# kartikmadhira1/YA_VO

Hardware: AMD Instinct MI355X
Metric: frames/sec (detect+describe+match+PnP) on 1241×376 KITTI stereo; RMSE vs CPU ref (higher is better)
Workload: dtype u8

## Files before the change

### ya_vo_amd/csrc/yavo_kernels.hip

```cpp
#include <hip/hip_runtime.h>
#include <stdint.h>
#include <stdlib.h>
#include <string.h>

#include <algorithm>

#include "yavo_xlane.h"
#include "yavo_internal.h"


namespace yavo {

__device__ __forceinline__ int lane_id() { return (int)(threadIdx.x & 63); }

__device__ __forceinline__ int wave_incl_scan(int v) {
    v += __builtin_amdgcn_update_dpp(0, v, 0x111, 0xf, 0xf, false);
    v += __builtin_amdgcn_update_dpp(0, v, 0x112, 0xf, 0xf, false);
    v += __builtin_amdgcn_update_dpp(0, v, 0x114, 0xf, 0xf, false);
    v += __builtin_amdgcn_update_dpp(0, v, 0x118, 0xf, 0xf, false);
    v += __builtin_amdgcn_update_dpp(0, v, 0x142, 0xa, 0xf, false);
    v += __builtin_amdgcn_update_dpp(0, v, 0x143, 0xc, 0xf, false);
    return v;
}

// ... 54 lines not shown
    float d0 = m00 / scale, d1 = m11 / scale, e = m01 / scale;
    int iter = 0, ok = 1;
    while (true) {
        if (fabsf(e) < 1.17549435082228750797e-38f) {
            e = 0.0f;
        } else {
            const float se = 8388608.0f * e;
            if (se * se <= (fabsf(d0) + fabsf(d1))) e = 0.0f;
        }
        if (e == 0.0f) break;
        if (++iter > 60) { ok = 0; break; }
        const float td = (d0 - d1) * 0.5f;
        float mu = d1;
        if (td == 0.0f) {
            mu -= fabsf(e);
        } else {
            const float e2 = e * e;
            const float h = eig_hypotf(td, e);
            if (e2 == 0.0f) mu -= e / ((td + (td > 0.0f ? h : -h)) / e);
            else mu -= e2 / (td + (td > 0.0f ? h : -h));
        }
        const float x = d0 - mu, z = e;
        float c, sn;
        if (x == 0.0f) {
            c = 0.0f;
            sn = z < 0.0f ? 1.0f : -1.0f;
        } else if (fabsf(x) > fabsf(z)) {
            const float t = z / x;
            float u = sqrtf(1.0f + t * t);
            if (x < 0.0f) u = -u;
            c = 1.0f / u;
            sn = -t * c;
        } else {
            const float t = x / z;
            float u = sqrtf(1.0f + t * t);
            if (z < 0.0f) u = -u;
            sn = -1.0f / u;
            c = -t * sn;
        }
        const float sdk = sn * d0 + c * e;
        const float dkp1 = sn * e + c * d1;
        const float nd0 = c * (c * d0 - sn * e) - sn * (c * e - sn * d1);
        const float nd1 = sn * sdk + c * dkp1;
        const float ne = c * sdk - sn * dkp1;
        d0 = nd0;
        d1 = nd1;
        e = ne;
    }
    if (ok && d1 < d0) { const float t = d0; d0 = d1; d1 = t; }
    d0 *= scale;
    d1 *= scale;
    w0 = d1;
    w1 = d0;
}

__device__ __forceinline__ float harris_response(float a, float b, float d, int eig) {
    float w0 = a, w1 = d;
    if (eig == 1) {
        eig_selfadjoint2(a, b, d, w0, w1);
    } else if (!(fabsf(b) <= 1.1920928955078125e-07f)) {
        const float p = b;
        const float y = (float)((double)(w1 - w0) * 0.5);
        float t = fabsf(y) + cv_hypotf(p, y);
        float s = cv_hypotf(p, t);
        s = p / s;
        t = (p / t) * p;
        if (y < 0.0f) { s = -s; t = -t; }
        w0 -= t;
        w1 += t;
    }
    if (eig != 1 && w0 < w1) { float tmp = w0; w0 = w1; w1 = tmp; }
    const float prod = w0 * w1;
    const float sum = w1 + w0;
    const double sq = (double)sum * (double)sum;
    const double r = (double)prod - 0.04 * sq;
    return (float)r;
}

__device__ __forceinline__ uint64_t make_key(float resp, uint32_t idx) {
    if (resp == 0.0f) resp = 0.0f;
    uint32_t u = __float_as_uint(resp);
    uint32_t ord = (u & 0x80000000u) ? ~u : (u | 0x80000000u);
    return ((uint64_t)(~ord) << 32) | (uint64_t)idx;
}
__device__ __forceinline__ float key_resp(uint64_t key) {
    uint32_t ord = ~(uint32_t)(key >> 32);
    uint32_t u = (ord & 0x80000000u) ? (ord & 0x7fffffffu) : ~ord;
    return __uint_as_float(u);
}

struct K9 {
    uint32_t k[9];
    uint32_t kh[4][3];
    int hbias;
};

static K9 make_k9(const uint16_t* k9) {
    K9 kw = {};
    uint32_t sum = 0;
    for (int i = 0; i < 9; ++i) {
        kw.k[i] = k9[i];
        sum += k9[i];
    }
    auto tap = [&](int t) -> uint32_t { return (t >= 0 && t <= 8) ? (uint32_t)k9[t] : 0u; };
    for (int j = 0; j < 4; ++j)
        for (int m = 0; m < 3; ++m)
            for (int i = 0; i < 4; ++i) kw.kh[j][m] |= tap(4 * m + i - j) << (8 * i);
    kw.hbias = (int)(128 * sum);
    return kw;
}

__device__ __forceinline__ int reflect101(int p, int len) {
    if (p < 0) p = -p;
    if (p >= len) p = 2 * len - p - 2;
    return p;
}

#ifdef YAVO_LM_PROFILE
constexpr int kDetProfSlots = 131072;
__device__ unsigned long long g_det_prof[kDetProfSlots][6];
#define DP_DECL unsigned long long dp_acc[6] = {0, 0, 0, 0, 0, 0}; unsigned long long dp_t = __builtin_readcyclecounter();
#define DP_MARK(k) do { const unsigned long long t_ = __builtin_readcyclecounter(); dp_acc[k] += t_ - dp_t; dp_t = t_; } while (0)
#define DP_STORE() do { \
        const unsigned slot_ = blockIdx.x; \
        if (threadIdx.x == 0 && slot_ < kDetProfSlots) for (int q_ = 0; q_ < 6; ++q_) g_det_prof[slot_][q_] = dp_acc[q_]; \
    } while (0)
constexpr int kBriefProfSlots = 16384;
__device__ unsigned long long g_brief_prof[kBriefProfSlots][6];
#define BP_DECL unsigned long long bp_acc[3] = {0, 0, 0}; unsigned long long bp_t = __builtin_readcyclecounter(); \
    unsigned long long bp_bands = 0; const unsigned long long bp_rt0 = __builtin_amdgcn_s_memrealtime();
#define BP_MARK(k) do { const unsigned long long t_ = __builtin_readcyclecounter(); bp_acc[k] += t_ - bp_t; bp_t = t_; } while (0)
#define BP_BAND() do { ++bp_bands; } while (0)
#define BP_STORE() do { \
        if (threadIdx.x == 0 && blockIdx.x < kBriefProfSlots) { \
            g_brief_prof[blockIdx.x][0] = bp_acc[0]; g_brief_prof[blockIdx.x][1] = bp_acc[1]; \
            g_brief_prof[blockIdx.x][2] = bp_rt0; \
            g_brief_prof[blockIdx.x][3] = __builtin_amdgcn_s_memrealtime(); \
            g_brief_prof[blockIdx.x][4] = (unsigned long long)__builtin_amdgcn_s_getreg(0xF804) | (bp_bands << 32); \
            g_brief_prof[blockIdx.x][5] = (unsigned long long)__builtin_amdgcn_s_getreg(0xF814) | (bp_acc[2] << 32); \
        } \
    } while (0)
#else
#define DP_DECL
#define DP_MARK(k) do {} while (0)
#define DP_STORE() do {} while (0)
#define BP_DECL
#define BP_MARK(k) do {} while (0)
#define BP_BAND() do {} while (0)
#define BP_STORE() do {} while (0)
#endif
constexpr int FT_W = kFastTileW;
constexpr int FT_H = kFastTileH;
constexpr int FT_R = 4;
constexpr int FT_LW = FT_W + 2 * FT_R;
constexpr int FT_LH = FT_H + 2 * FT_R;
constexpr int kBandM = 19;
constexpr int kBlurStageDw = FT_LH * (FT_W / 4);

__device__ __forceinline__ void blur_tile_mfma(const uint8_t* tile, const uint32_t* s_band, uint32_t* stage, int hbias,
                                               int lane, int cb) {
    typedef int dt_v4i __attribute__((ext_vector_type(4)));
    const int nn = lane & 15, g = lane >> 4;
    const uint32_t* band = &s_band[(nn & 3) * kBandM + 3 - (nn >> 2)];
    const dt_v4i B = {(int)band[4 * g], (int)band[4 * g + 1], (int)band[4 * g + 2], (int)band[4 * g + 3]};
    const dt_v4i Z = {0, 0, 0, 0};
    const uint8_t* arow = &tile[nn * FT_LW + 16 * cb + 16 * g];
    dt_v4i Hlo, Hhi;
#pragma unroll
    for (int rb = 0; rb < 4; ++rb) {
        const uint2 lo = *reinterpret_cast<const uint2*>(arow + 16 * rb * FT_LW);
        const uint2 hi = *reinterpret_cast<const uint2*>(arow + 16 * rb * FT_LW + 8);
        const dt_v4i A = {(int)(lo.x ^ 0x80808080u), (int)(lo.y ^ 0x80808080u), (int)(hi.x ^ 0x80808080u),
                          (int)(hi.y ^ 0x80808080u)};
        const dt_v4i acc = __builtin_amdgcn_mfma_i32_16x16x64_i8(A, B, Z, 0, 0, 0);
        const uint32_t p01 = __builtin_amdgcn_perm((uint32_t)acc[1], (uint32_t)acc[0], 0x05010400u);
        const uint32_t p23 = __builtin_amdgcn_perm((uint32_t)acc[3], (uint32_t)acc[2], 0x05010400u);
        Hlo[rb] = (int)(__builtin_amdgcn_perm(p23, p01, 0x05040100u) ^ 0x80808080u);
        Hhi[rb] = (int)__builtin_amdgcn_perm(p23, p01, 0x07060302u);
    }
    const int T0 = (int)band[g], T1 = (int)band[g + 4];
    const int cv = 257 * hbias + (1 << 15);
    const dt_v4i Cv = {cv, cv, cv, cv};
    uint32_t* ostage = &stage[nn * 16 + ((4 * cb) ^ (nn & 12)) + g];
#pragma unroll
    for (int ob = 0; ob < 4; ++ob) {
        dt_v4i T = {0, 0, 0, 0};
        T[ob] = T0;
        if (ob < 3) T[ob + 1] = T1;
        const dt_v4i vl = __builtin_amdgcn_mfma_i32_16x16x64_i8(Hlo, T, Cv, 0, 0, 0);
        const dt_v4i vh = __builtin_amdgcn_mfma_i32_16x16x64_i8(Hhi, T, Z, 0, 0, 0);
        uint32_t v[4];
#pragma unroll
        for (int i = 0; i < 4; ++i) v[i] = ((uint32_t)vh[i] << 8) + (uint32_t)vl[i];
        ostage[ob * 16 * 16] = __builtin_amdgcn_perm(__builtin_amdgcn_perm(v[3], v[2], 0x0c0c0602u),
                                                     __builtin_amdgcn_perm(v[1], v[0], 0x0c0c0602u), 0x05040100u);
    }
}

__device__ __forceinline__ void blur_store_rows(const uint32_t* stage, uint8_t* __restrict__ blur, int img, int H, int W,
                                                int r0, int c0, int tid) {
    if (tid < FT_H * 4) {
        const int R = tid >> 2, q = tid & 3;
        const int bp = blur_pitch(W);
        if (r0 + R < H)
            *reinterpret_cast<uint4*>(blur + ((int64_t)img * H + r0 + R) * bp + c0 + 16 * (q ^ ((R >> 2) & 3))) =
                *reinterpret_cast<const uint4*>(&stage[R * 16 + 4 * q]);
    }
}

template <bool kBlur>
__global__ __launch_bounds__(256) void detect_kernel(const uint8_t* __restrict__ imgs, int H, int W, int stride,
                                                     int64_t pitch, int thr, int eig, uint64_t* __restrict__ cand_keys,
                                                     int64_t cap, uint32_t* __restrict__ cand_count, K9 kw,
                                                     uint8_t* __restrict__ blur) {
    __shared__ __align__(16) uint8_t tile[FT_LH * FT_LW];
    constexpr int kPreDw = FT_W * FT_H / 2;
    static_assert(kBlurStageDw <= kPreDw, "the blur's output staging must fit in the pretest list");
    __shared__ __align__(16) uint32_t s_share[kPreDw];
    uint16_t* s_pre = reinterpret_cast<uint16_t*>(s_share);
    __shared__ uint16_t s_pos[FT_W * FT_H];
    __shared__ uint32_t s_n, s_npre, s_base;
    __shared__ uint32_t s_band[4 * kBandM];
    DP_DECL
    const int ntx = (W + FT_W - 1) / FT_W, nty = (H + FT_H - 1) / FT_H;
    const int lb = xcd_swizzle((int)blockIdx.x, (int)gridDim.x);
    const int img = lb / (ntx * nty), tyx = lb - img * (ntx * nty);
    const int r0 = (tyx / ntx) * FT_H, c0 = (tyx % ntx) * FT_W;
    const uint8_t* src = imgs + (int64_t)img * pitch;
    const int tid = threadIdx.x;
    const int lane = lane_id();
    const int wave = tid >> 6;
    if (tid == 0) {
        s_n = 0;
        s_npre = 0;
    }
    if (kBlur && tid < 4 * kBandM) {
        const int r = tid / kBandM, M = tid - kBandM * r - 3;
        uint32_t v = 0;
#pragma unroll
        for (int j = 0; j < 4; ++j)
#pragma unroll
            for (int m = 0; m < 3; ++m)
                if (r == j && M == m) v = kw.kh[j][m];
        s_band[tid] = v;
    }

    {
        constexpr int kDw = FT_LW / 4;
        constexpr int kSlots = FT_LH * kDw;
        constexpr int kPer = (kSlots + 255) / 256;
        const bool interior = (c0 >= FT_R) && (c0 + FT_W + FT_R <= W) && (r0 >= FT_R) && (r0 + FT_H + FT_R < H);
        uint32_t v[kPer];
        if (interior) {
            const uint8_t* base = src + (int64_t)(r0 - FT_R) * stride + (c0 - FT_R);
            const int lr0 = tid / kDw, j0 = tid - lr0 * kDw;
            uint32_t off = (uint32_t)(lr0 * stride + 4 * j0);
            int j = j0;
            const uint32_t step = (uint32_t)(14 * stride + 16), wrap = (uint32_t)(15 * stride - 56);
            const uint32_t last = (uint32_t)((kSlots - 1) / kDw * stride + 4 * ((kSlots - 1) % kDw));
#pragma unroll
            for (int u = 0; u < kPer; ++u) {
                const uint32_t o = (256 * u + 255 >= kSlots && tid + 256 * u >= kSlots) ? last : off;
                __builtin_memcpy(&v[u], base + o, 4);
                const bool c = j + 4 >= kDw;
                off += c ? wrap : step;
                j += c ? 4 - kDw : 4;
            }
        } else {
#pragma unroll
            for (int u = 0; u < kPer; ++u) {
                const int t = min(tid + 256 * u, kSlots - 1);
                const int lr = t / kDw, j = t - lr * kDw;
                const int r = reflect101(min(max(r0 - FT_R + lr, -(H - 1)), 2 * H - 2), H);
                const uint8_t* row = src + (int64_t)r * stride;
                const int cc = c0 - FT_R + 4 * j;
                if (cc >= 0 && cc + 4 <= W) {
                    __builtin_memcpy(&v[u], row + cc, 4);
                } else {
                    uint32_t w = 0;
#pragma unroll
                    for (int b = 0; b < 4; ++b)
                        w |= (uint32_t)row[reflect101(min(max(cc + b, -(W - 1)), 2 * W - 2), W)] << (8 * b);
                    v[u] = w;
                }
            }
        }
        uint32_t* tile32 = reinterpret_cast<uint32_t*>(tile);
#pragma unroll
        for (int u = 0; u < kPer; ++u) {
            const int t = tid + 256 * u;
            if (t < kSlots) tile32[t] = v[u];
        }
    }
    __syncthreads();
    DP_MARK(0);

    constexpr int ring_dr[16] = YV_RING_DR;
    constexpr int ring_dc[16] = YV_RING_DC;
    const uint32_t neg_thr = (uint32_t)(-thr);
    const int tx = lane;
    const int ty = __builtin_amdgcn_readfirstlane(wave);
    const int c = c0 + tx;
    constexpr int kRowIters = FT_H / 4;
    uint32_t row_ok = 0;
#pragma unroll
    for (int u = 0; u < kRowIters; ++u) row_ok |= (uint32_t)((unsigned)(r0 + ty + 4 * u - 4) < (unsigned)(H - 8)) << u;
    uint32_t nmask = 0;
    const uint8_t* wbase = &tile[(ty + FT_R - 3) * FT_LW + tx + FT_R - 3];
#pragma unroll
    for (int u = kRowIters - 1; u >= 0; --u) {
        const uint8_t* t0 = wbase + 4 * u * FT_LW;
        const uint32_t cent = t0[3 * FT_LW + 3];
        auto d = [&](int k) {
            return __builtin_amdgcn_sad_u8(cent, (uint32_t)t0[(ring_dr[k] + 3) * FT_LW + ring_dc[k] + 3], neg_thr);
        };
        const uint32_t v = (d(0) | d(4)) | (d(8) | d(11));
        nmask = __builtin_amdgcn_alignbit(nmask, v, 31);
    }
    uint32_t pmask = (unsigned)(c - 4) < (unsigned)(W - 8) ? (~nmask & row_ok) : 0u;
    {
        const int cnt = __popc(pmask);
        const int incl = wave_incl_scan(cnt);
        const int total = __shfl(incl, 63, 64);
        uint32_t base = 0;
        if (lane == 0 && total > 0) base = atomicAdd(&s_npre, (uint32_t)total);
        base = __shfl(base, 0, 64);
        uint32_t off = base + (uint32_t)(incl - cnt);
        while (pmask) {
            const int u = __builtin_ctz(pmask);
            s_pre[off++] = (uint16_t)((ty + 4 * u) * FT_W + tx);
            pmask &= pmask - 1;
        }
    }
    __syncthreads();
    DP_MARK(1);
    const uint32_t npre = s_npre;
    for (uint32_t i0 = 0; i0 < npre; i0 += 256) {
        const uint32_t i = i0 + tid;
        bool cand = false;
        int pos = 0;
        if (i < npre) {
            pos = s_pre[i];
            const uint8_t* t0 = &tile[((pos >> 6) + FT_R - 3) * FT_LW + (pos & 63) + FT_R - 3];
            const uint32_t cent = t0[3 * FT_LW + 3];
            uint32_t sim = 0;
#pragma unroll
            for (int k = 0; k < 16; ++k)
                sim = __builtin_amdgcn_alignbit(
                    sim, __builtin_amdgcn_sad_u8(cent, (uint32_t)t0[(ring_dr[k] + 3) * FT_LW + ring_dc[k] + 3], neg_thr),
                    31);
            const uint32_t mask = ~sim & 0xFFFFu;
            const uint32_t a2 = mask & (mask >> 1);
            const uint32_t a4 = a2 & (a2 >> 2);
            const uint32_t a8 = a4 & (a4 >> 4);
            const uint32_t a12 = a8 & (a4 >> 8);
            cand = a12 != 0u;
        }
        const uint64_t bal = __ballot(cand);
        if (bal == 0) continue;
        const int leader = __ffsll((long long)bal) - 1;
        uint32_t base = 0;
        if (lane == leader) base = atomicAdd(&s_n, (uint32_t)__popcll(bal));
        base = __shfl(base, leader, 64);
        if (cand) s_pos[base + (uint32_t)__popcll(bal & ((1ull << lane) - 1ull))] = (uint16_t)pos;
    }
    __syncthreads();
    DP_MARK(2);
    const uint32_t n = s_n;
    auto harris = [&](uint32_t base) {
        uint64_t* out = cand_keys + (int64_t)img * cap + base;
        for (uint32_t i = tid; i < n; i += 256) {
            const int pos = s_pos[i];
            const int prr = pos >> 6, ptx = pos & 63;
            const uint8_t* t0 = &tile[(prr + FT_R - 2) * FT_LW + ptx + FT_R - 2];
            int sxx = 0, sxy = 0, syy = 0;
#pragma unroll
            for (int ii = -1; ii <= 1; ++ii) {
#pragma unroll
                for (int j = -1; j <= 1; ++j) {
                    const uint8_t* q = t0 + (ii + 2) * FT_LW + j + 2;
                    const int pmm = q[-FT_LW - 1], pm0 = q[-FT_LW], pmp = q[-FT_LW + 1];
                    const int p0m = q[-1], p0p = q[1];
                    const int ppm = q[FT_LW - 1], pp0 = q[FT_LW], ppp = q[FT_LW + 1];
                    const int gx = (pmp - pmm) + 2 * (p0p - p0m) + (ppp - ppm);
                    const int gy = (ppm - pmm) + 2 * (pp0 - pm0) + (ppp - pmp);
                    sxx += gx * gx;
                    sxy += gx * gy;
                    syy += gy * gy;
                }
            }
            const float resp = harris_response((float)sxx, (float)sxy, (float)syy, eig);
            out[i] = make_key(resp, (uint32_t)((r0 + prr) * W + (c0 + ptx)));
        }
    };
    if (tid == 0 && n > 0) s_base = atomicAdd(&cand_count[img], n);
    if constexpr (kBlur) blur_tile_mfma(tile, s_band, s_share, kw.hbias, lane, ty);
    __syncthreads();
    if constexpr (kBlur) blur_store_rows(s_share, blur, img, H, W, r0, c0, tid);
    DP_MARK(3);
    if (n > 0) harris(s_base);
    DP_MARK(4);
    DP_STORE();
}

void launch_fast_harris(const uint8_t* imgs, int n_images, int H, int W, int stride, int64_t pitch,
                        int thr, int eig, uint64_t* cand_keys, int64_t cap, uint32_t* cand_count, hipStream_t s) {
    dim3 grid(((W + FT_W - 1) / FT_W) * ((H + FT_H - 1) / FT_H) * n_images);
    K9 kw = {};
    hipLaunchKernelGGL(detect_kernel<false>, grid, dim3(256), 0, s, imgs, H, W, stride, pitch, thr, eig, cand_keys,
                       cap, cand_count, kw, (uint8_t*)nullptr);
}

void launch_detect_blur(const uint8_t* imgs, int n_images, int H, int W, int stride, int64_t pitch, int thr,
                        int eig, uint64_t* cand_keys, int64_t cap, uint32_t* cand_count, const uint16_t* k9_host,
                        uint8_t* blur, hipStream_t s) {
    uint32_t max_tap = 0;
    for (int i = 0; i < 9; ++i) max_tap = k9_host[i] > max_tap ? k9_host[i] : max_tap;
    if (max_tap > 127) {
        launch_fast_harris(imgs, n_images, H, W, stride, pitch, thr, eig, cand_keys, cap, cand_count, s);
        launch_blur9(imgs, n_images, H, W, stride, pitch, k9_host, blur, s);
        return;
    }
    dim3 grid(((W + FT_W - 1) / FT_W) * ((H + FT_H - 1) / FT_H) * n_images);
    const K9 kw = make_k9(k9_host);
    hipLaunchKernelGGL(detect_kernel<true>, grid, dim3(256), 0, s, imgs, H, W, stride, pitch, thr, eig, cand_keys, cap,
                       cand_count, kw, blur);
}

constexpr int BL_W = 64, BL_H = 32, BL_R = 4;
constexpr int BL_LW = BL_W + 2 * BL_R;
constexpr int BL_LH = BL_H + 2 * BL_R;

__global__ __launch_bounds__(256) void blur9_kernel(const uint8_t* __restrict__ imgs, int H, int W, int stride,
                                                    int64_t pitch, K9 kw, uint8_t* __restrict__ blur) {
    __shared__ uint8_t tin[BL_LH * BL_LW];
    __shared__ uint32_t th[BL_LH * BL_W];
    const int img = blockIdx.z;
    const int r0 = blockIdx.y * BL_H, c0 = blockIdx.x * BL_W;
    const uint8_t* src = imgs + (int64_t)img * pitch;
    const int tid = threadIdx.x;
    for (int i = tid; i < BL_LH * BL_LW; i += 256) {
        const int lr = i / BL_LW, lc = i - lr * BL_LW;
        const int r = reflect101(min(max(r0 - BL_R + lr, -(H - 1)), 2 * H - 2), H);
        const int c = reflect101(min(max(c0 - BL_R + lc, -(W - 1)), 2 * W - 2), W);
        tin[i] = src[(int64_t)r * stride + c];
    }
    __syncthreads();
    for (int i = tid; i < BL_LH * BL_W; i += 256) {
        const int lr = i >> 6, lc = i & 63;
        const uint8_t* q = &tin[lr * BL_LW + lc];
        uint32_t acc = 0;
#pragma unroll
        for (int j = 0; j < 9; ++j) acc += kw.k[j] * (uint32_t)q[j];
        th[i] = acc;
    }
    __syncthreads();
    const int tx = tid & 63, ty = tid >> 6;
    const int c = c0 + tx;
    for (int rr = ty; rr < BL_H; rr += 4) {
        const int r = r0 + rr;
        uint32_t acc = 0;
#pragma unroll
        for (int i = 0; i < 9; ++i) acc += kw.k[i] * th[(rr + i) * BL_W + tx];
        uint32_t v = (acc + (1u << 15)) >> 16;
        if (r < H && c < W) blur[(int64_t)img * blur_image_bytes(H, W) + (int64_t)r * blur_pitch(W) + c] = (uint8_t)(v > 255u ? 255u : v);
    }
}

void launch_blur9(const uint8_t* imgs, int n_images, int H, int W, int stride, int64_t pitch,
                  const uint16_t* k9_host, uint8_t* blur, hipStream_t s) {
    const K9 kw = make_k9(k9_host);
    constexpr int kMaxGridZ = 65535;
    for (int i0 = 0; i0 < n_images; i0 += kMaxGridZ) {
        const int n = n_images - i0 < kMaxGridZ ? n_images - i0 : kMaxGridZ;
        dim3 grid((W + BL_W - 1) / BL_W, (H + BL_H - 1) / BL_H, n);
        hipLaunchKernelGGL(blur9_kernel, grid, dim3(256), 0, s, imgs + (int64_t)i0 * pitch, H, W, stride, pitch, kw,
                           blur + (int64_t)i0 * blur_image_bytes(H, W));
    }
}

constexpr int TK_NT = 1024;

__device__ __forceinline__ bool brief_boundary(int row, int col, int H, int W) {
    return !(col - 8 < 0 || col + 8 > W) && !(row - 8 < 0 || row + 8 > H);
}

__host__ __device__ constexpr int bank_classes(int nb) { return nb <= kBandCounters / 32 ? 32 : 1; }

template <int NT, class RcAt>
__device__ void boundary_compact(RcAt rc_at, int K, int H, int W, int32_t* kp_src, int32_t* kp_count,
                                 int32_t* kp_band, int32_t* band_off, int* s_tmp, int* s_band) {
    const int tid = threadIdx.x;
    const int nb = (H + kBandRows - 1) / kBandRows;
    const int C = bank_classes(nb), nbc = nb * C;
    const int LS = brief_lds_stride(W);
    auto bucket = [&](int row, int col) -> int {
        const int band = row / kBandRows;
        const int cls = C == 1 ? 0 : ((((row - band * kBandRows + 8) * LS + col) >> 2) & 31);
        return band * C + cls;
    };
    for (int b = tid; b < nbc; b += NT) s_band[b] = 0;
    __syncthreads();
    int base = 0;
    for (int pass = 0; pass < 2; ++pass) {
        base = 0;
        for (int c0 = 0; c0 < K; c0 += 4 * NT) {
            int flags[4];
            int2 rcs[4];
            int cnt = 0;
#pragma unroll
            for (int u = 0; u < 4; ++u) {
                const int i = c0 + tid * 4 + u;
                flags[u] = 0;
                rcs[u] = make_int2(0, 0);
                if (i < K) {
                    rcs[u] = rc_at(i);
                    flags[u] = brief_boundary(rcs[u].x, rcs[u].y, H, W) ? 1 : 0;
                }
                cnt += flags[u];
            }
            int total = 0;
            int off = base + block_excl_scan<NT>(cnt, s_tmp, &total);
#pragma unroll
            for (int u = 0; u < 4; ++u) {
                const int i = c0 + tid * 4 + u;
                if (flags[u]) {
                    const int bk = bucket(rcs[u].x, rcs[u].y);
                    if (pass == 0) {
                        reinterpret_cast<int4*>(kp_src)[off] = make_int4(rcs[u].x, rcs[u].y, i, 0);
                        atomicAdd(&s_band[bk], 1);
                    } else {
                        const int pos = atomicAdd(&s_band[bk], 1);
                        reinterpret_cast<int4*>(kp_band)[pos] = make_int4(rcs[u].x, rcs[u].y, i, off);
                    }
                    off++;
                }
            }
            base += total;
        }
        __syncthreads();
        if (pass == 0) {
            int acc = 0;
            for (int b0 = 0; b0 < nbc; b0 += NT) {
                const int j = b0 + tid;
                const int c = j < nbc ? s_band[j] : 0;
                int tot = 0;
                const int first = acc + block_excl_scan<NT>(c, s_tmp, &tot);
                if (j < nbc) {
                    s_band[j] = first;
                    if (j % C == 0) band_off[j / C] = first;
                }
                acc += tot;
            }
            if (tid == 0) band_off[nb] = acc;
        }
        __syncthreads();
    }
    if (tid == 0) *kp_count = base;
}

constexpr int TK_SEL_NT = 512;
static_assert(TK_SEL_NT >= 256 && TK_SEL_NT % 64 == 0, "the radix-select histogram scan uses the first 256 threads");
template <int NT>
__global__ __launch_bounds__(NT) void topk_kernel(const uint64_t* __restrict__ cand_keys, int64_t cap,
                                                     uint32_t* __restrict__ cand_count, uint32_t* __restrict__ cand_seen,
                                                     int H, int W, int max_kp, int keep, int32_t* __restrict__ det_rc,
                                                     float* __restrict__ det_resp, int32_t* __restrict__ det_count,
                                                     int32_t* __restrict__ kp_src, int32_t* __restrict__ kp_count,
                                                     int32_t* __restrict__ kp_band, int32_t* __restrict__ band_off,
                                                     int32_t* __restrict__ brief_heads) {
    __shared__ uint64_t s_keys[kMaxKp];
    __shared__ uint32_t s_hist[256];
    __shared__ int s_tmp[40];
    __shared__ int s_band[kBandCounters];
    __shared__ uint64_t s_prefix, s_mask;
    __shared__ int s_krem, s_done, s_n;

    const int img = blockIdx.x;
    const int tid = threadIdx.x;
    if (img == 0 && tid < kBriefHeads) brief_heads[tid] = 0;
    const uint64_t* keys = cand_keys + (int64_t)img * cap;
    int64_t C64 = (int64_t)cand_count[img];
    if (C64 > cap) C64 = cap;
    const int C = (int)C64;
    const int K = C < keep ? C : keep;
    __syncthreads();
    if (tid == 0) {
        cand_seen[img] = (uint32_t)C;
        cand_count[img] = 0;
    }
    int32_t* rc_out = det_rc + (int64_t)img * max_kp * 2;
    float* resp_out = det_resp + (int64_t)img * max_kp;

    if (K == 0) {
        const int nb = (H + kBandRows - 1) / kBandRows;
        for (int b = tid; b <= nb; b += NT) band_off[(int64_t)img * (kMaxBands + 1) + b] = 0;
        if (tid == 0) { det_count[img] = 0; kp_count[img] = 0; }
        return;
    }
    uint64_t sel_mask = 0, sel_prefix = ~0ull;
    if (C > K) {
        if (tid == 0) { s_prefix = 0; s_mask = 0; s_krem = K; s_done = 0; }
        __syncthreads();
        for (int shift = 56; shift >= 0; shift -= 8) {
            const uint64_t pm = s_mask, pp = s_prefix;
            const int krem = s_krem;
            if (tid < 256) s_hist[tid] = 0;
            __syncthreads();
            for (int i = tid; i < C; i += NT) {
                const uint64_t k = keys[i];
                if ((k & pm) == pp) atomicAdd(&s_hist[(k >> shift) & 255u], 1u);
            }
            __syncthreads();
            int h = 0, incl = 0;
            if (tid < 256) {
                h = (int)s_hist[tid];
                incl = wave_incl_scan(h);
                if ((tid & 63) == 63) s_tmp[tid >> 6] = incl;
            }
            __syncthreads();
            if (tid < 256) {
                int base = 0;
                for (int w = 0; w < (tid >> 6); ++w) base += s_tmp[w];
                incl += base;
                if (incl >= krem && incl - h < krem) {
                    const int nk = krem - (incl - h);
                    s_prefix = pp | ((uint64_t)tid << shift);
                    s_mask = pm | (0xFFull << shift);
                    s_krem = nk;
                    s_done = (h == nk);
                }
            }
            __syncthreads();
// ... 1008 lines not shown
```

Measured before the change: 253,600.

## Reassign FAST pretest rows to contiguous blocks and reuse ring pixels across rows

Each wave now owns a contiguous block of rows instead of interleaved rows, so the vertical ring samples (offsets 0/8) are loaded once into registers and reused across neighbouring rows. The horizontal sample is derived by shifting the sim8 mask across lanes with DPP row shifts, and a ballot-based halo computation covers the three edge lanes. This cuts LDS loads per candidate in the pretest stage. It also replaces the shfl broadcasts with readlane/readfirstlane, at the cost of more complex lane-dependent logic whose correctness at block edges depends on the DPP and halo mapping.

```diff
diff --git a/ya_vo_amd/csrc/yavo_kernels.hip b/ya_vo_amd/csrc/yavo_kernels.hip
--- a/ya_vo_amd/csrc/yavo_kernels.hip
+++ b/ya_vo_amd/csrc/yavo_kernels.hip
@@ -380,33 +380,55 @@
     const int ty = __builtin_amdgcn_readfirstlane(wave);
     const int c = c0 + tx;
     constexpr int kRowIters = FT_H / 4;
+    static_assert(4 * kRowIters == FT_H && kRowIters <= 16, "four row blocks; the halo round packs 16 rows a column");
+    const int rb = kRowIters * ty;
     uint32_t row_ok = 0;
 #pragma unroll
-    for (int u = 0; u < kRowIters; ++u) row_ok |= (uint32_t)((unsigned)(r0 + ty + 4 * u - 4) < (unsigned)(H - 8)) << u;
-    uint32_t nmask = 0;
-    const uint8_t* wbase = &tile[(ty + FT_R - 3) * FT_LW + tx + FT_R - 3];
-#pragma unroll
-    for (int u = kRowIters - 1; u >= 0; --u) {
-        const uint8_t* t0 = wbase + 4 * u * FT_LW;
-        const uint32_t cent = t0[3 * FT_LW + 3];
-        auto d = [&](int k) {
-            return __builtin_amdgcn_sad_u8(cent, (uint32_t)t0[(ring_dr[k] + 3) * FT_LW + ring_dc[k] + 3], neg_thr);
-        };
-        const uint32_t v = (d(0) | d(4)) | (d(8) | d(11));
-        nmask = __builtin_amdgcn_alignbit(nmask, v, 31);
-    }
-    uint32_t pmask = (unsigned)(c - 4) < (unsigned)(W - 8) ? (~nmask & row_ok) : 0u;
+    for (int u = 0; u < kRowIters; ++u) row_ok |= (uint32_t)((unsigned)(r0 + rb + u - 4) < (unsigned)(H - 8)) << u;
+    uint32_t sim411 = 0, sim8 = 0;
+    {
+        const uint8_t* wbase = &tile[(rb + FT_R - 3) * FT_LW + tx + FT_R];
+        uint32_t o[kRowIters + 3], rt[kRowIters], tp[kRowIters];
+#pragma unroll
+        for (int k = 0; k < kRowIters + 3; ++k) o[k] = wbase[(k + 3) * FT_LW];
+#pragma unroll
+        for (int k = 0; k < kRowIters; ++k) {
+            rt[k] = wbase[(k + 3) * FT_LW + 3];
+            tp[k] = wbase[k * FT_LW + 1];
+        }
+#pragma unroll
+        for (int u = kRowIters - 1; u >= 0; --u) {
+            const uint32_t cent = o[u];
+            const uint32_t v = __builtin_amdgcn_sad_u8(cent, o[u + 3], neg_thr) |
+                               __builtin_amdgcn_sad_u8(cent, tp[u], neg_thr);
+            sim411 = __builtin_amdgcn_alignbit(sim411, v, 31);
+            sim8 = __builtin_amdgcn_alignbit(sim8, __builtin_amdgcn_sad_u8(cent, rt[u], neg_thr), 31);
+        }
+    }
+    uint32_t sim0 = sim8;
+#pragma unroll
+    for (int i = 0; i < 3; ++i) sim0 = (uint32_t)__builtin_amdgcn_update_dpp(0, (int)sim0, 0x138, 0xf, 0xf, true);
+    {
+        const uint8_t* q = &tile[(rb + FT_R) * FT_LW + FT_R - 3] + (__umul24(lane & 15, FT_LW) + (lane >> 4));
+        const uint64_t hal = __ballot((int)__builtin_amdgcn_sad_u8((uint32_t)q[0], (uint32_t)q[3], neg_thr) < 0);
+        if (lane < 3) sim0 = (uint32_t)(hal >> (16 * lane)) & ((1u << kRowIters) - 1u);
+    }
+    uint32_t pmask = (unsigned)(c - 4) < (unsigned)(W - 8) ? (~(sim411 | sim8 | sim0) & row_ok) : 0u;
     {
         const int cnt = __popc(pmask);
         const int incl = wave_incl_scan(cnt);
-        const int total = __shfl(incl, 63, 64);
+        const int total = __builtin_amdgcn_readlane(incl, 63);
         uint32_t base = 0;
-        if (lane == 0 && total > 0) base = atomicAdd(&s_npre, (uint32_t)total);
-        base = __shfl(base, 0, 64);
+        if (total > 0) {
+            uint32_t add = (uint32_t)total;
+            asm volatile("" : "+v"(add));
+            if (lane == 0) base = atomicAdd(&s_npre, add);
+            base = (uint32_t)__builtin_amdgcn_readfirstlane((int)base);
+        }
         uint32_t off = base + (uint32_t)(incl - cnt);
         while (pmask) {
             const int u = __builtin_ctz(pmask);
-            s_pre[off++] = (uint16_t)((ty + 4 * u) * FT_W + tx);
+            s_pre[off++] = (uint16_t)((rb + u) * FT_W + tx);
             pmask &= pmask - 1;
         }
     }
```

After: 252,200, median of 3. No clear change (-0.6%).
